# lz4/lz4-java

Measured on NVIDIA H100. Metric: lz4_fast_compress_plus_decompress_64KiB_blocks, higher is better.
Workload: dtype u8

## Files before the change

lz4-java_b200/csrc/lz4_decompress.cu:

```cuda
#include "common.cuh"
#include "kernels.h"

namespace b200 {

#ifndef B200_DEC_MINB_BATCH
#define B200_DEC_MINB_BATCH 8
#endif
#ifndef B200_DEC_WIN
#define B200_DEC_WIN 512
#endif
static constexpr int DEC_WIN = B200_DEC_WIN;

struct VarLen { uint32_t len; int ip; bool err; };

__device__ __forceinline__ VarLen read_varlen(const uint8_t* __restrict__ src, int ip, int ilimit, bool initial_check)
{
    VarLen r; r.len = 0; r.ip = ip; r.err = false;
    if (initial_check && ip >= ilimit) { r.err = true; return r; }
    uint32_t s;
    do {
        s = src[r.ip]; r.ip++;
        r.len = min(r.len + s, 0x40000000u);
        if (r.ip > ilimit) { r.err = true; return r; }
    } while (s == 255);
    return r;
}

__device__ __forceinline__ void lane_copy16(uint8_t* d, const uint8_t* s, int n)
{
    const uintptr_t sa = reinterpret_cast<uintptr_t>(s);
    const uint32_t* w = reinterpret_cast<const uint32_t*>(sa & ~uintptr_t(3));
    const uint32_t sh = (uint32_t(sa) & 3u) * 8u;
    uint32_t x[5];
    #pragma unroll
    for (int t = 0; t < 5; t++) x[t] = (4 * t < n + 3) ? w[t] : 0u;
    #pragma unroll
    for (int t = 0; t < 4; t++) {
        const uint32_t v = __funnelshift_r(x[t], x[t + 1], sh);
        if (4 * t     < n) d[4 * t]     = uint8_t(v);
        if (4 * t + 1 < n) d[4 * t + 1] = uint8_t(v >> 8);
        if (4 * t + 2 < n) d[4 * t + 2] = uint8_t(v >> 16);
        if (4 * t + 3 < n) d[4 * t + 3] = uint8_t(v >> 24);
    }
}

__device__ __forceinline__ int decode_batch(const uint8_t* __restrict__ src, uint8_t* dst, int& ip, int& op,
                                            const int iend, const int oend, const int lane, uint8_t* win)
{
    const uint8_t* __restrict__ in = src + ip;
    uint8_t* cls = win + DEC_WIN;
    {
        const uintptr_t base = reinterpret_cast<uintptr_t>(in);
        const uint32_t* __restrict__ W = reinterpret_cast<const uint32_t*>(base & ~uintptr_t(3)) + 4 * lane;
        const uint32_t a8 = (uint32_t(base) & 3u) * 8u;
        const uint32_t w0 = W[0], w1 = W[1], w2 = W[2], w3 = W[3], w4 = W[4];
        uint32_t f[4];
        f[0] = __funnelshift_r(w0, w1, a8); f[1] = __funnelshift_r(w1, w2, a8); f[2] = __funnelshift_r(w2, w3, a8); f[3] = __funnelshift_r(w3, w4, a8);
        uint32_t c[4];
        #pragma unroll
        for (int k = 0; k < 4; k++) {
            const uint32_t t = f[k];
            const uint32_t lit = (t >> 4) & 0x0F0F0F0Fu, ml = t & 0x0F0F0F0Fu;
            const uint32_t m15 = ((ml + 0x01010101u) >> 4) & 0x01010101u;
            c[k] = (lit + 0x03030303u) | (m15 << 5);
        }
        __syncwarp();
        reinterpret_cast<uint4*>(win)[lane] = make_uint4(f[0], f[1], f[2], f[3]);
        reinterpret_cast<uint4*>(cls)[lane] = make_uint4(c[0], c[1], c[2], c[3]);
        __syncwarp();
    }
    auto wbyte = [&](int p) -> uint32_t { return p < DEC_WIN ? win[p] : in[p]; };
    const int ilim = iend - ip - 64;
    const int olim = oend - op - 128;

    int k = 0, q = 0;
    int m_tok = 0;
    while (k < 32 && q < DEC_WIN - 8) {
        const int c = cls[q];
        int s = c & 31;
        if (c > 17) {
            bool ok = true;
            if (s == 18) {
                int p = q + 1, lit = 15; uint32_t e;
                do { if (p >= ilim) { ok = false; break; } e = wbyte(p++); lit += int(e); } while (e == 255u && lit < (1 << 24));
                s = (p - q) + lit + 2;
                ok = ok && lit < (1 << 24);
            }
            if (ok && (c & 32)) {
                uint32_t e; int cnt = 0;
                do { if (q + s >= ilim) { ok = false; break; } e = wbyte(q + s); s++; } while (e == 255u && ++cnt < (1 << 16));
                ok = ok && cnt < (1 << 16);
            }
            if (!ok || q + s > ilim) break;
        }
        if (lane == k) m_tok = q;
        q += s; k++;
    }
    if (k == 0) return 0;
    int m_lit = 0, m_ml = 0, m_lsrc = 0;
    if (lane < k) {
        const uint32_t tok = win[m_tok];
        m_lit = int(tok >> 4); m_ml = int(tok & 15u) + 4; m_lsrc = m_tok + 1;
        if (m_lit == 15) { uint32_t e; do { e = wbyte(m_lsrc++); m_lit += int(e); } while (e == 255u); }
        if (m_ml == 19) { int p = m_lsrc + m_lit + 2; uint32_t e; do { e = wbyte(p++); m_ml += int(e); } while (e == 255u); }
    }
    int m_out = m_lit + m_ml;
    #pragma unroll
    for (int d = 1; d < 32; d <<= 1) { const int y = __shfl_up_sync(B200_FULL, m_out, d); if (lane >= d) m_out += y; }
    {
        const unsigned over = __ballot_sync(B200_FULL, lane < k && m_out > olim);
        if (over) {
            k = __ffs(over) - 1;
            if (k == 0) return 0;
            q = __shfl_sync(B200_FULL, m_tok, k);
        }
    }
    int acc = __shfl_sync(B200_FULL, m_out, k - 1);
    m_out -= m_lit + m_ml;
    if (lane >= k) { m_lit = 0; m_ml = 0; }

    int off = 1;
    if (lane < k) off = int(in[m_lsrc + m_lit]) | (int(in[m_lsrc + m_lit + 1]) << 8);
    const int mstart = op + m_out + m_lit;
    const unsigned bad = __ballot_sync(B200_FULL, lane < k && (off == 0 || off > mstart));
    if (bad) {
        k = __ffs(bad) - 1;
        if (k == 0) return 0;
        acc = __shfl_sync(B200_FULL, m_out, k);
        q = __shfl_sync(B200_FULL, m_tok, k);
    }
    const bool mine = lane < k;

    if (mine) lane_copy16(dst + op + m_out, in + m_lsrc, min(m_lit, 16));
    if (__any_sync(B200_FULL, mine && m_lit > 16)) {
        if (mine && m_lit > 16) lane_copy16(dst + op + m_out + 16, in + m_lsrc + 16, min(m_lit - 16, 16));
        for (unsigned lm = __ballot_sync(B200_FULL, mine && m_lit > 32); lm; lm &= lm - 1) {
            const int j = __ffs(lm) - 1;
            const int jo = __shfl_sync(B200_FULL, m_out, j), js = __shfl_sync(B200_FULL, m_lsrc, j), jl = __shfl_sync(B200_FULL, m_lit, j);
            warp_copy(dst + op + jo + 32, in + js + 32, jl - 32, lane);
        }
    }
    __syncwarp();

    const bool ovl = off < m_ml;
    const int mend = mstart - off + m_ml;
    unsigned pend = k == 32 ? B200_FULL : (1u << k) - 1u;
    while (pend) {
        const int fp = __ffs(pend) - 1;
        const int fpm = __shfl_sync(B200_FULL, mstart, fp);
        if (__shfl_sync(B200_FULL, int(ovl), fp)) {
            warp_match_copy(dst + fpm, __shfl_sync(B200_FULL, off, fp), __shfl_sync(B200_FULL, m_ml, fp), lane);
            pend &= pend - 1;
            __syncwarp();
            continue;
        }
        const bool ready = ((pend >> lane) & 1u) && !ovl && (lane == fp || mend <= fpm);
        const unsigned rm = __ballot_sync(B200_FULL, ready);
        if (ready) lane_copy16(dst + mstart, dst + mstart - off, min(m_ml, 16));
        if (__any_sync(B200_FULL, ready && m_ml > 16)) {
            if (ready && m_ml > 16) lane_copy16(dst + mstart + 16, dst + mstart - off + 16, min(m_ml - 16, 16));
            for (unsigned lm = __ballot_sync(B200_FULL, ready && m_ml > 32); lm; lm &= lm - 1) {
                const int j = __ffs(lm) - 1;
                const int jm = __shfl_sync(B200_FULL, mstart, j), jo = __shfl_sync(B200_FULL, off, j), jl = __shfl_sync(B200_FULL, m_ml, j);
                warp_copy(dst + jm + 32, dst + jm - jo + 32, jl - 32, lane);
            }
        }
        pend &= ~rm;
        __syncwarp();
    }
    ip += q; op += acc;
    return k;
}

template <int WARPS, bool BATCH>
__global__ void __launch_bounds__(WARPS * 32, BATCH ? B200_DEC_MINB_BATCH : 2048 / (WARPS * 32))
lz4_decompress_safe_kernel(const uint8_t* __restrict__ src_base, const uint64_t* __restrict__ src_off,
                           const int32_t* __restrict__ src_len,
                           uint8_t* dst_base, const uint64_t* __restrict__ dst_off,
                           const int32_t* __restrict__ dst_cap, int32_t* __restrict__ result, uint32_t n)
{
    __shared__ __align__(16) uint8_t s_win[BATCH ? WARPS : 1][2 * DEC_WIN];
    uint8_t* win = s_win[BATCH ? (threadIdx.x >> 5) : 0];
    const uint32_t b = blockIdx.x * WARPS + (threadIdx.x >> 5);
    if (b >= n) return;
    const int lane = lane_id();
    const uint8_t* __restrict__ src = src_base + src_off[b];
    uint8_t* dst = dst_base + dst_off[b];
    const int iend = src_len[b];
    const int oend = dst_cap[b];
    int ip = 0, op = 0;
    int ret;

    if (oend < 0) { ret = -1; goto done; }
    if (oend == 0) { ret = (iend == 1 && src[0] == 0) ? 0 : -1; goto done; }
    if (iend <= 0) { ret = -1; goto done; }
    {
        bool fastloop = oend >= 64;
        const uint8_t* __restrict__ sl = src + lane;
        uint8_t* dl = dst + lane;
        for (;;) {
            while (BATCH && fastloop && ip + DEC_WIN + 128 <= iend && op + 256 <= oend) { if (decode_batch(src, dst, ip, op, iend, oend, lane, win) == 0) break; }
            while (fastloop && ip + 18 <= iend) {
                const uint32_t token = src[ip];
                const uint32_t lit = token >> 4, mlc = token & 15;
                if (lit == 15 || mlc == 15) break;
                if (lane < lit) dl[op] = sl[ip + 1];
                const int ipo = ip + 1 + (int)lit;
                const uint32_t off = (uint32_t)src[ipo] | ((uint32_t)src[ipo + 1] << 8);
                const int op2 = op + (int)lit, ml = (int)mlc + 4;
                if (op2 + ml >= oend - 64 || off > (uint32_t)op2 || off == 0) break;
                __syncwarp();
                if (off >= (uint32_t)ml) { if (lane < ml) dl[op2] = dl[op2 - (int)off]; }
                else warp_match_copy(dst + op2, (int)off, ml, lane);
                ip = ipo + 2; op = op2 + ml;
            }
            const uint32_t token = src[ip++];
            uint32_t len = token >> 4;
            bool apply_end_rule, shortcut = false;
            if (fastloop) {
                bool leave;
                if (len == 15) {
                    VarLen v = read_varlen(src, ip, iend - 15, true);
                    ip = v.ip; if (v.err) goto error;
                    len += v.len;
                    leave = ((long long)op + len > oend - 32) || ((long long)ip + len > iend - 32);
                } else leave = ip > iend - 17;
                if (leave) fastloop = false;
                apply_end_rule = leave;
            } else {
                shortcut = (len != 15) && (ip < iend - 16) && (op <= oend - 32);
                if (!shortcut && len == 15) {
                    VarLen v = read_varlen(src, ip, iend - 15, true);
                    ip = v.ip; if (v.err) goto error;
                    len += v.len;
                }
                apply_end_rule = !shortcut;
            }
            const long long lcpy = (long long)op + len;
            if (apply_end_rule && (lcpy > oend - 12 || (long long)ip + len > iend - 8)) {
                if ((long long)ip + len != iend || lcpy > oend) goto error;
                warp_copy(dst + op, src + ip, (int)len, lane);
                op += (int)len;
                break;
            }
            warp_copy(dst + op, src + ip, (int)len, lane);
            ip += (int)len; op += (int)len;

            const int off = src[ip] | (src[ip + 1] << 8);
            ip += 2;
            uint32_t ml = token & 15;
            const bool direct = shortcut && ml != 15 && off >= 8 && off <= op;
            if (ml == 15) {
                VarLen v = read_varlen(src, ip, iend - 4, false);
                ip = v.ip; if (v.err) goto error;
                ml += v.len;
            }
            ml += 4;
            if (!direct) {
                if (off > op) goto error;
                const long long mcpy = (long long)op + ml;
                if (fastloop && mcpy >= oend - 64) fastloop = false;
                if (mcpy > oend - 5) goto error;
            }
            __syncwarp();
            if (off == 0) {
                for (int i = lane; i < (int)ml; i += 32) dst[op + i] = 0;
            } else {
                warp_match_copy(dst + op, off, (int)ml, lane);
            }
            op += (int)ml;
        }
        ret = op;
        goto done;
    }
error:
    ret = -ip - 1;
done:
    __syncwarp();
    if (lane == 0) { __threadfence(); result[b] = ret; }
}

template <int WARPS, bool BATCH>
__global__ void __launch_bounds__(WARPS * 32, BATCH ? B200_DEC_MINB_BATCH : 2048 / (WARPS * 32))
lz4_decompress_fast_kernel(const uint8_t* __restrict__ src_base, const uint64_t* __restrict__ src_off,
                           const int32_t* __restrict__ src_avail,
                           uint8_t* dst_base, const uint64_t* __restrict__ dst_off,
                           const int32_t* __restrict__ dst_len, int32_t* __restrict__ result, uint32_t n)
{
    __shared__ __align__(16) uint8_t s_win[BATCH ? WARPS : 1][2 * DEC_WIN];
    uint8_t* win = s_win[BATCH ? (threadIdx.x >> 5) : 0];
    const uint32_t b = blockIdx.x * WARPS + (threadIdx.x >> 5);
    if (b >= n) return;
    const int lane = lane_id();
    const uint8_t* __restrict__ src = src_base + src_off[b];
    uint8_t* dst = dst_base + dst_off[b];
    const int avail = src_avail[b];
    const int oend = dst_len[b];
    int ip = 0, op = 0, ret = -1;

    if (oend < 0) goto done;
    for (;;) {
        while (BATCH && ip + DEC_WIN + 128 <= avail && op + 256 <= oend) { if (decode_batch(src, dst, ip, op, avail, oend, lane, win) == 0) break; }
        {
            const uint8_t* __restrict__ sl = src + lane;
            uint8_t* dl = dst + lane;
            while (ip + 17 <= avail) {
                const uint32_t token = src[ip];
                const uint32_t lit = token >> 4, mlc = token & 15;
                if (lit == 15 || mlc == 15) break;
                const int op2 = op + (int)lit, ml = (int)mlc + 4;
                if (op2 + 23 > oend) break;
                if (lane < lit) dl[op] = sl[ip + 1];
                const int ipo = ip + 1 + (int)lit;
                const uint32_t off = (uint32_t)src[ipo] | ((uint32_t)src[ipo + 1] << 8);
                if (off > (uint32_t)op2 || off == 0) break;
                __syncwarp();
                if (off >= (uint32_t)ml) { if (lane < ml) dl[op2] = dl[op2 - (int)off]; }
                else warp_match_copy(dst + op2, (int)off, ml, lane);
                ip = ipo + 2; op = op2 + ml;
            }
        }
        if (ip >= avail) goto done;
        const uint32_t token = src[ip++];
        uint32_t ll = token >> 4;
        if (ll == 15) {
            uint32_t s;
            do { if (ip >= avail) goto done; s = src[ip++]; ll = min(ll + s, 0x40000000u); } while (s == 255);
        }
        if ((uint32_t)(oend - op) < ll) goto done;
        if ((long long)ip + ll > avail) goto done;
        warp_copy(dst + op, src + ip, (int)ll, lane);
        op += (int)ll; ip += (int)ll;
        if (oend - op < 12) {
            if (op == oend) { ret = ip; }
            goto done;
        }
        if (ip + 2 > avail) goto done;
        const int off = src[ip] | (src[ip + 1] << 8);
        ip += 2;
        uint32_t ml = token & 15;
        if (ml == 15) {
            uint32_t s;
            do { if (ip >= avail) goto done; s = src[ip++]; ml = min(ml + s, 0x40000000u); } while (s == 255);
        }
        ml += 4;
        if ((uint32_t)(oend - op) < ml) goto done;
        if (off > op) goto done;
        __syncwarp();
        if (off != 0) warp_match_copy(dst + op, off, (int)ml, lane);
        else for (int i = lane; i < (int)ml; i += 32) dst[op + i] = 0;
        op += (int)ml;
        if (oend - op < 5) goto done;
    }
done:
    if (lane == 0) result[b] = ret;
}

#ifndef B200_HOST_SIM
static constexpr int DEC_WARPS = 4;

cudaError_t launch_decompress_safe(const BatchArgs& a, cudaStream_t st)
{
    if (a.n == 0) return cudaSuccess;
    const unsigned grid = (unsigned)((a.n + DEC_WARPS - 1) / DEC_WARPS);
    lz4_decompress_safe_kernel<DEC_WARPS, true><<<grid, DEC_WARPS * 32, 0, st>>>(
        a.src_base, a.src_off, a.src_len, a.dst_base, a.dst_off, a.dst_cap, a.result, (uint32_t)a.n);
    return cudaGetLastError();
}

cudaError_t launch_decompress_fast(const BatchArgs& a, cudaStream_t st)
{
    if (a.n == 0) return cudaSuccess;
    const unsigned grid = (unsigned)((a.n + DEC_WARPS - 1) / DEC_WARPS);
    lz4_decompress_fast_kernel<DEC_WARPS, true><<<grid, DEC_WARPS * 32, 0, st>>>(
        a.src_base, a.src_off, a.src_len, a.dst_base, a.dst_off, a.dst_cap, a.result, (uint32_t)a.n);
    return cudaGetLastError();
}

#endif

}
```

lz4-java_b200/csrc/xxhash.cu:

```cuda
#include "common.cuh"
#include "kernels.h"

namespace b200 {

static constexpr uint32_t P32_1 = 2654435761u, P32_2 = 2246822519u, P32_3 = 3266489917u,
                          P32_4 = 668265263u, P32_5 = 374761393u;
static constexpr uint64_t P64_1 = 11400714785074694791ull, P64_2 = 14029467366897019727ull,
                          P64_3 = 1609587929392839161ull, P64_4 = 9650029242287828579ull,
                          P64_5 = 2870177450012600261ull;

__device__ __forceinline__ uint32_t rotl32(uint32_t x, int r) { return __funnelshift_l(x, x, r); }
__device__ __forceinline__ uint64_t rotl64(uint64_t x, int r) { return (x << r) | (x >> (64 - r)); }
__device__ __forceinline__ uint32_t round32(uint32_t acc, uint32_t w) { return rotl32(acc + w * P32_2, 13) * P32_1; }
__device__ __forceinline__ uint64_t round64(uint64_t acc, uint64_t w) { return rotl64(acc + w * P64_2, 31) * P64_1; }
__device__ __forceinline__ uint64_t merge64(uint64_t h, uint64_t v) { return (h ^ round64(0, v)) * P64_1 + P64_4; }

__device__ __forceinline__ uint64_t load_u64_unaligned(const uint8_t* p)
{
    return uint64_t(load_u32_unaligned(p)) | (uint64_t(load_u32_unaligned(p + 4)) << 32);
}

__device__ __forceinline__ uint32_t finish32(uint32_t h, const uint8_t* p, uint32_t rem)
{
    while (rem >= 4) { h = rotl32(h + load_u32_unaligned(p) * P32_3, 17) * P32_4; p += 4; rem -= 4; }
    while (rem)      { h = rotl32(h + uint32_t(*p++) * P32_5, 11) * P32_1; rem--; }
    h ^= h >> 15; h *= P32_2; h ^= h >> 13; h *= P32_3; h ^= h >> 16;
    return h;
}
__device__ __forceinline__ uint64_t finish64(uint64_t h, const uint8_t* p, uint32_t rem)
{
    while (rem >= 8) { h = rotl64(h ^ round64(0, load_u64_unaligned(p)), 27) * P64_1 + P64_4; p += 8; rem -= 8; }
    if (rem >= 4)    { h = rotl64(h ^ (uint64_t(load_u32_unaligned(p)) * P64_1), 23) * P64_2 + P64_3; p += 4; rem -= 4; }
    while (rem)      { h = rotl64(h ^ (uint64_t(*p++) * P64_5), 11) * P64_1; rem--; }
    h ^= h >> 33; h *= P64_2; h ^= h >> 29; h *= P64_3; h ^= h >> 32;
    return h;
}

#ifndef B200_HOST_SIM
__device__ __forceinline__ uint32_t smem_u32(const void* p) { return (uint32_t)__cvta_generic_to_shared(p); }
__device__ __forceinline__ void mbar_init(uint32_t bar, uint32_t count)
{ asm volatile("mbarrier.init.shared::cta.b64 [%0], %1;" :: "r"(bar), "r"(count) : "memory"); }
__device__ __forceinline__ void mbar_arrive_expect_tx(uint32_t bar, uint32_t bytes)
{ asm volatile("mbarrier.arrive.expect_tx.shared::cta.b64 _, [%0], %1;" :: "r"(bar), "r"(bytes) : "memory"); }
__device__ __forceinline__ void mbar_wait(uint32_t bar, uint32_t parity)
{
    uint32_t ok;
    do {
        asm volatile("{\n\t.reg .pred p;\n\tmbarrier.try_wait.parity.shared::cta.b64 p, [%1], %2;\n\tselp.u32 %0, 1, 0, p;\n\t}"
                     : "=r"(ok) : "r"(bar), "r"(parity) : "memory");
    } while (!ok);
}
__device__ __forceinline__ void tma_bulk_g2s(uint32_t dst_smem, const void* src_gmem, uint32_t bytes, uint32_t bar)
{
    asm volatile("cp.async.bulk.shared::cluster.global.mbarrier::complete_tx::bytes [%0], [%1], %2, [%3];"
                 :: "r"(dst_smem), "l"(src_gmem), "r"(bytes), "r"(bar) : "memory");
}

#endif

template <int BITS> struct XxhTraits;
template <> struct XxhTraits<32> { using word = uint32_t; static constexpr int STRIPE = 16; };
template <> struct XxhTraits<64> { using word = uint64_t; static constexpr int STRIPE = 32; };

template <int BITS> struct Acc;
template <> struct Acc<32> {
    uint32_t v1, v2, v3, v4;
    __device__ __forceinline__ void init(uint32_t seed) { v1 = seed + P32_1 + P32_2; v2 = seed + P32_2; v3 = seed; v4 = seed - P32_1; }
    __device__ __forceinline__ void stripe(uint4 q) { v1 = round32(v1, q.x); v2 = round32(v2, q.y); v3 = round32(v3, q.z); v4 = round32(v4, q.w); }
    __device__ __forceinline__ void stripe_g(const uint8_t* p) {
        stripe(make_uint4(load_u32_unaligned(p), load_u32_unaligned(p + 4), load_u32_unaligned(p + 8), load_u32_unaligned(p + 12)));
    }
    __device__ __forceinline__ uint32_t merge() const { return rotl32(v1, 1) + rotl32(v2, 7) + rotl32(v3, 12) + rotl32(v4, 18); }
};
template <> struct Acc<64> {
    uint64_t v1, v2, v3, v4;
    __device__ __forceinline__ void init(uint64_t seed) { v1 = seed + P64_1 + P64_2; v2 = seed + P64_2; v3 = seed; v4 = seed - P64_1; }
    __device__ __forceinline__ void stripe(uint4 a, uint4 b) {
        v1 = round64(v1, uint64_t(a.x) | (uint64_t(a.y) << 32)); v2 = round64(v2, uint64_t(a.z) | (uint64_t(a.w) << 32));
        v3 = round64(v3, uint64_t(b.x) | (uint64_t(b.y) << 32)); v4 = round64(v4, uint64_t(b.z) | (uint64_t(b.w) << 32));
    }
    __device__ __forceinline__ void stripe_g(const uint8_t* p) {
        v1 = round64(v1, load_u64_unaligned(p)); v2 = round64(v2, load_u64_unaligned(p + 8));
        v3 = round64(v3, load_u64_unaligned(p + 16)); v4 = round64(v4, load_u64_unaligned(p + 24));
    }
    __device__ __forceinline__ uint64_t merge() const {
        uint64_t h = rotl64(v1, 1) + rotl64(v2, 7) + rotl64(v3, 12) + rotl64(v4, 18);
        h = merge64(h, v1); h = merge64(h, v2); h = merge64(h, v3); h = merge64(h, v4);
        return h;
    }
};

#ifndef B200_HOST_SIM
static constexpr int XXH_WARPS = 4;
static constexpr int XXH_CHUNK = 256;
static constexpr int XXH_SLOT  = XXH_CHUNK + 16;
static constexpr int XXH_STAGES = 2;
static constexpr size_t XXH_SMEM = size_t(XXH_WARPS) * XXH_STAGES * 32 * XXH_SLOT + 64;

template <int BITS>
__global__ void __launch_bounds__(XXH_WARPS * 32)
xxh_batch_kernel(const uint8_t* __restrict__ base, const uint64_t* __restrict__ off, const int32_t* __restrict__ len,
                 typename XxhTraits<BITS>::word seed, typename XxhTraits<BITS>::word* __restrict__ out, uint32_t n)
{
    using word = typename XxhTraits<BITS>::word;
    constexpr int STRIPE = XxhTraits<BITS>::STRIPE;
    extern __shared__ __align__(128) uint8_t smem[];
    const int warp = threadIdx.x >> 5, lane = lane_id();
    const uint32_t first = (blockIdx.x * XXH_WARPS + warp) * 32;
    if (first >= n) return;
    const uint32_t i = first + lane;
    const bool live = i < n;

    const uint8_t* p = live ? base + off[i] : base;
    const uint32_t L = live ? (uint32_t)max(len[i], 0) : 0u;
    const uint32_t bulk = L & ~uint32_t(STRIPE - 1);
    Acc<BITS> acc; acc.init(seed);

    uint64_t* bars = reinterpret_cast<uint64_t*>(smem);
    uint8_t* slots = smem + 64 + size_t(warp) * XXH_STAGES * 32 * XXH_SLOT;
    const bool aligned = (reinterpret_cast<uintptr_t>(p) & 15) == 0 || bulk == 0;

    if (__all_sync(B200_FULL, aligned)) {
        const uint32_t bar0 = smem_u32(&bars[warp * XXH_STAGES]);
        if (lane == 0) {
            for (int s = 0; s < XXH_STAGES; s++) mbar_init(bar0 + 8 * s, 1);
            asm volatile("fence.mbarrier_init.release.cluster;" ::: "memory");
        }
        __syncwarp();
        const uint32_t nchunks = (bulk + XXH_CHUNK - 1) / XXH_CHUNK;
        const uint32_t maxchunks = __reduce_max_sync(B200_FULL, nchunks);

        auto issue = [&](uint32_t k) {
            const uint32_t s = k % XXH_STAGES;
            const uint32_t bytes = k < nchunks ? min(uint32_t(XXH_CHUNK), bulk - k * XXH_CHUNK) : 0u;
            const uint32_t total = __reduce_add_sync(B200_FULL, bytes);
            if (lane == 0) mbar_arrive_expect_tx(bar0 + 8 * s, total);
            if (bytes) tma_bulk_g2s(smem_u32(slots + (size_t(s) * 32 + lane) * XXH_SLOT), p + size_t(k) * XXH_CHUNK, bytes, bar0 + 8 * s);
        };
        for (uint32_t k = 0; k < XXH_STAGES && k < maxchunks; k++) issue(k);
        for (uint32_t k = 0; k < maxchunks; k++) {
            const uint32_t s = k % XXH_STAGES;
            mbar_wait(bar0 + 8 * s, (k / XXH_STAGES) & 1);
            if (k < nchunks) {
                const uint32_t bytes = min(uint32_t(XXH_CHUNK), bulk - k * XXH_CHUNK);
                const uint4* q = reinterpret_cast<const uint4*>(slots + (size_t(s) * 32 + lane) * XXH_SLOT);
                if constexpr (BITS == 32) {
                    #pragma unroll 4
                    for (uint32_t j = 0; j < bytes / 16; j++) acc.stripe(q[j]);
                } else {
                    #pragma unroll 4
                    for (uint32_t j = 0; j < bytes / 32; j++) acc.stripe(q[2 * j], q[2 * j + 1]);
                }
            }
            __syncwarp();
            if (k + XXH_STAGES < maxchunks) issue(k + XXH_STAGES);
        }
    } else {
        for (uint32_t o = 0; o < bulk; o += STRIPE) acc.stripe_g(p + o);
    }

    if (live) {
        if constexpr (BITS == 32) {
            uint32_t h = (L >= 16u) ? acc.merge() : seed + P32_5;
            out[i] = finish32(h + L, p + bulk, L - bulk);
        } else {
            uint64_t h = (L >= 32u) ? acc.merge() : seed + P64_5;
            out[i] = finish64(h + uint64_t(L), p + bulk, L - bulk);
        }
    }
}

cudaError_t launch_xxh32(const uint8_t* base, const uint64_t* off, const int32_t* len, uint32_t seed,
                         uint32_t* out, size_t n, cudaStream_t st)
{
    if (n == 0) return cudaSuccess;
    auto k = xxh_batch_kernel<32>;
    cudaError_t e = cudaFuncSetAttribute(k, cudaFuncAttributeMaxDynamicSharedMemorySize, (int)XXH_SMEM);
    if (e != cudaSuccess) return e;
    const unsigned grid = (unsigned)((n + XXH_WARPS * 32 - 1) / (XXH_WARPS * 32));
    k<<<grid, XXH_WARPS * 32, XXH_SMEM, st>>>(base, off, len, seed, out, (uint32_t)n);
    return cudaGetLastError();
}

cudaError_t launch_xxh64(const uint8_t* base, const uint64_t* off, const int32_t* len, uint64_t seed,
                         uint64_t* out, size_t n, cudaStream_t st)
{
    if (n == 0) return cudaSuccess;
    auto k = xxh_batch_kernel<64>;
    cudaError_t e = cudaFuncSetAttribute(k, cudaFuncAttributeMaxDynamicSharedMemorySize, (int)XXH_SMEM);
    if (e != cudaSuccess) return e;
    const unsigned grid = (unsigned)((n + XXH_WARPS * 32 - 1) / (XXH_WARPS * 32));
    k<<<grid, XXH_WARPS * 32, XXH_SMEM, st>>>(base, off, len, seed, out, (uint32_t)n);
    return cudaGetLastError();
}

#endif

__device__ __forceinline__ uint32_t xxh32_chain_init(uint32_t seed, int lane)
{
    const int c = lane & 3;
    return c == 0 ? seed + P32_1 + P32_2 : c == 1 ? seed + P32_2 : c == 2 ? seed : seed - P32_1;
}

template <bool CG>
__device__ __forceinline__ uint32_t xxh_ldw(const uint32_t* p)
{
#ifndef B200_HOST_SIM
    if constexpr (CG) return __ldcg(p);
#endif
    return *p;
}

template <bool CG = false>
__device__ __forceinline__ uint32_t xxh32_warp_rows(uint32_t v, const uint8_t* __restrict__ p, size_t rows, int lane)
{
    constexpr int R = 8;
    const uintptr_t sa = reinterpret_cast<uintptr_t>(p);
    const uint32_t* __restrict__ W = reinterpret_cast<const uint32_t*>(sa & ~uintptr_t(3));
    const uint32_t sh = (uint32_t(sa) & 3u) * 8u;
    const int c = lane & 3;
    auto ldrow = [&](size_t r) -> uint32_t {
        const size_t i = r * 32 + lane;
        const uint32_t a = xxh_ldw<CG>(W + i);
        return sh ? __funnelshift_r(a, xxh_ldw<CG>(W + i + 1), sh) : a;
    };
    uint32_t cur[R], nxt[R];
    const size_t groups = rows / R;
    if (groups) {
        #pragma unroll
        for (int r = 0; r < R; r++) cur[r] = ldrow(r);
    }
    for (size_t g = 0; g < groups; g++) {
        if (g + 1 < groups) {
            #pragma unroll
            for (int r = 0; r < R; r++) nxt[r] = ldrow((g + 1) * R + r);
        }
        #pragma unroll
        for (int r = 0; r < R; r++) {
            #pragma unroll
            for (int st = 0; st < 8; st++) v = round32(v, __shfl_sync(B200_FULL, cur[r], 4 * st + c));
        }
        #pragma unroll
        for (int r = 0; r < R; r++) cur[r] = nxt[r];
    }
    for (size_t r = groups * R; r < rows; r++) {
        const uint32_t x = ldrow(r);
        #pragma unroll
        for (int st = 0; st < 8; st++) v = round32(v, __shfl_sync(B200_FULL, x, 4 * st + c));
    }
    return v;
}

template <bool CG = false>
__device__ __forceinline__ uint32_t xxh32_warp_stripes(uint32_t v, const uint8_t* __restrict__ p, size_t stripes, int lane)
{
    const size_t rows = stripes >> 3;
    v = xxh32_warp_rows<CG>(v, p, rows, lane);
    for (size_t t = rows << 3; t < stripes; t++) {
        const uint8_t* q = p + 16 * t + 4 * (lane & 3);
        if constexpr (CG) {
            const uintptr_t a = reinterpret_cast<uintptr_t>(q);
            const uint32_t* w = reinterpret_cast<const uint32_t*>(a & ~uintptr_t(3));
            const uint32_t sh = (uint32_t(a) & 3u) * 8u;
            const uint32_t lo = xxh_ldw<true>(w);
            v = round32(v, sh ? __funnelshift_r(lo, xxh_ldw<true>(w + 1), sh) : lo);
        } else {
            v = round32(v, load_u32_unaligned(q));
        }
    }
    return v;
}

__device__ __forceinline__ uint32_t xxh32_chain_merge(uint32_t v)
{
    return rotl32(__shfl_sync(B200_FULL, v, 0), 1) + rotl32(__shfl_sync(B200_FULL, v, 1), 7) +
           rotl32(__shfl_sync(B200_FULL, v, 2), 12) + rotl32(__shfl_sync(B200_FULL, v, 3), 18);
}

__global__ void __launch_bounds__(32)
xxh32_long_kernel(const uint8_t* __restrict__ base, const uint64_t* __restrict__ off, const int32_t* __restrict__ len,
                  uint32_t seed, uint32_t* __restrict__ out, uint32_t n)
{
    const uint32_t i = blockIdx.x;
    if (i >= n) return;
    const int lane = lane_id();
    const uint8_t* __restrict__ p = base + off[i];
    const uint32_t L = (uint32_t)max(len[i], 0);
    const size_t stripes = L >> 4;
    uint32_t h;
    if (L >= 16u) h = xxh32_chain_merge(xxh32_warp_stripes(xxh32_chain_init(seed, lane), p, stripes, lane));
    else h = seed + P32_5;
    if (lane == 0) out[i] = finish32(h + L, p + 16 * stripes, L & 15u);
}

#ifndef B200_HOST_SIM
cudaError_t launch_xxh32_long(const uint8_t* base, const uint64_t* off, const int32_t* len, uint32_t seed,
                              uint32_t* out, size_t n, cudaStream_t st)
{
    if (n == 0) return cudaSuccess;
    xxh32_long_kernel<<<(unsigned)n, 32, 0, st>>>(base, off, len, seed, out, (uint32_t)n);
    return cudaGetLastError();
}
#endif

__global__ void __launch_bounds__(32)
xxh32_long_carry_kernel(const uint8_t* __restrict__ base, const uint64_t* __restrict__ off, const uint64_t* __restrict__ len,
                        uint32_t* __restrict__ out, Xxh32Carry* __restrict__ c_state, const uint8_t* __restrict__ c_mode, uint32_t n)
{
    __shared__ __align__(16) uint8_t s_mem[16];
    const uint32_t r = blockIdx.x;
    if (r >= n) return;
    const int lane = lane_id();
    const uint32_t mode = c_mode[r];
    const uint8_t* __restrict__ p = base + off[r];
    uint64_t L = len[r];
    uint32_t v = xxh32_chain_init(0u, lane), mem = 0;
    uint64_t total = 0;
    if (mode & XXH_CARRY_IN) {
        const Xxh32Carry& c = c_state[r];
        v = c.v[lane & 3]; total = c.total; mem = c.memsize;
        if (uint32_t(lane) < mem) s_mem[lane] = c.mem[lane];
    }
    __syncwarp();
    total += L;
    if (mem + L < 16u) {
        if (uint32_t(lane) < L) s_mem[mem + lane] = p[lane];
        mem += (uint32_t)L; L = 0;
    } else {
        if (mem) {
            const uint32_t t = 16u - mem;
            if (uint32_t(lane) < t) s_mem[mem + lane] = p[lane];
            __syncwarp();
            v = round32(v, reinterpret_cast<const uint32_t*>(s_mem)[lane & 3]);
            p += t; L -= t; mem = 0;
            __syncwarp();
        }
        const size_t stripes = size_t(L >> 4);
        v = xxh32_warp_stripes(v, p, stripes, lane);
        mem = uint32_t(L & 15u);
        if (uint32_t(lane) < mem) s_mem[lane] = p[16 * stripes + lane];
    }
    __syncwarp();
    if (mode & XXH_CARRY_OUT) {
        Xxh32Carry& c = c_state[r];
        if (lane < 4) c.v[lane] = v;
        if (uint32_t(lane) < mem) c.mem[lane] = s_mem[lane];
        if (lane == 0) { c.total = total; c.memsize = mem; }
        return;
    }
    const uint32_t h = total >= 16 ? xxh32_chain_merge(v) : 0u + P32_5;
    if (lane == 0) out[r] = finish32(h + uint32_t(total), s_mem, mem);
}

cudaError_t launch_xxh32_long_carry(const uint8_t* base, const uint64_t* off, const uint64_t* len, uint32_t* out, Xxh32Carry* carry,
                                    const uint8_t* mode, size_t n, cudaStream_t st)
{
    if (n == 0) return cudaSuccess;
    B200_LAUNCH(xxh32_long_carry_kernel, (unsigned)n, 32, st, base, off, len, out, carry, mode, (uint32_t)n);
    return cudaGetLastError();
}

__device__ __forceinline__ uint8_t ld_byte_l2(const uint8_t* p)
{
#ifndef B200_HOST_SIM
    return __ldcg(p);
#else
    return *p;
#endif
}

__global__ void __launch_bounds__(32)
xxh32_frames_chained_kernel(const uint8_t* __restrict__ slots, const uint64_t* __restrict__ blk_off, const uint32_t* __restrict__ f_first,
                            const uint32_t* __restrict__ f_nblk, const int32_t* __restrict__ blk_comp, const int32_t* __restrict__ blk_rawlen,
                            const int32_t* c_res, uint32_t* __restrict__ out, uint32_t n, Xxh32Carry* c_state = nullptr,
                            const uint8_t* c_mode = nullptr)
{
    __shared__ __align__(16) uint8_t s_carry[16];
    const uint32_t f = blockIdx.x;
    if (f >= n) return;
    const int lane = lane_id();
    const uint32_t first = f_first[f], nblk = f_nblk[f];
    const uint32_t mode = c_mode ? c_mode[f] : 0u;
    uint32_t v = xxh32_chain_init(0u, lane);
    uint64_t total = 0; uint32_t carry = 0;
    bool big = false;
    if (mode & XXH_CARRY_IN) {
        const Xxh32Carry& c = c_state[f];
        v = c.v[lane & 3]; total = c.total; carry = c.memsize; big = total >= 16;
        if (uint32_t(lane) < carry) s_carry[lane] = c.mem[lane];
        __syncwarp();
    }
    for (uint32_t k = 0; k < nblk; k++) {
        const int32_t ci = blk_comp[first + k];
        int32_t r;
        if (ci < 0) r = blk_rawlen[first + k];
        else {
            const volatile int32_t* w = c_res + ci;
            r = 0;
            if (lane == 0) { while ((r = *w) == FRAME_RES_PENDING) { B200_NANOSLEEP(256); } }
            r = __shfl_sync(B200_FULL, r, 0);
            __threadfence();
            if (r < 0) break;
        }
        const uint8_t* p = slots + blk_off[first + k];
        uint32_t len = uint32_t(r);
        total += len;
        if (carry) {
            const uint32_t t = min(16u - carry, len);
            if (uint32_t(lane) < t) s_carry[carry + lane] = ld_byte_l2(p + lane);
            __syncwarp();
            carry += t; p += t; len -= t;
            if (carry < 16u) continue;
            v = round32(v, reinterpret_cast<const uint32_t*>(s_carry)[lane & 3]); big = true; carry = 0;
            __syncwarp();
        }
        const size_t stripes = size_t(len) >> 4;
        if (stripes) { v = xxh32_warp_stripes<true>(v, p, stripes, lane); big = true; }
        carry = len & 15u;
        if (uint32_t(lane) < carry) s_carry[lane] = ld_byte_l2(p + 16 * stripes + lane);
        __syncwarp();
    }
    if (mode & XXH_CARRY_OUT) {
        Xxh32Carry& c = c_state[f];
        if (lane < 4) c.v[lane] = v;
        if (uint32_t(lane) < carry) c.mem[lane] = s_carry[lane];
        if (lane == 0) { c.total = total; c.memsize = carry; }
        return;
    }
    const uint32_t h = big ? xxh32_chain_merge(v) : 0u + P32_5;
    if (lane == 0) out[f] = finish32(h + uint32_t(total), s_carry, carry);
}

#ifndef B200_HOST_SIM
cudaError_t launch_xxh32_frames_chained(const uint8_t* slots, const uint64_t* blk_off, const uint32_t* f_first, const uint32_t* f_nblk,
                                        const int32_t* blk_comp, const int32_t* blk_rawlen, const int32_t* c_res,
                                        uint32_t* out, size_t n, cudaStream_t st)
{
    if (n == 0) return cudaSuccess;
    xxh32_frames_chained_kernel<<<(unsigned)n, 32, 0, st>>>(slots, blk_off, f_first, f_nblk, blk_comp, blk_rawlen, c_res, out, (uint32_t)n);
    return cudaGetLastError();
}
#endif
cudaError_t launch_xxh32_frames_chained_carry(const uint8_t* slots, const uint64_t* blk_off, const uint32_t* f_first,
                                              const uint32_t* f_nblk, const int32_t* blk_comp, const int32_t* blk_rawlen,
                                              const int32_t* c_res, uint32_t* out, size_t n, Xxh32Carry* carry,
                                              const uint8_t* mode, cudaStream_t st)
{
    if (n == 0) return cudaSuccess;
    B200_LAUNCH(xxh32_frames_chained_kernel, (unsigned)n, 32, st, slots, blk_off, f_first, f_nblk, blk_comp, blk_rawlen, c_res, out,
                (uint32_t)n, carry, mode);
    return cudaGetLastError();
}

__device__ __forceinline__ uint64_t xxh64_chain_init(uint64_t seed, int lane)
{
    const int c = lane & 3;
    return c == 0 ? seed + P64_1 + P64_2 : c == 1 ? seed + P64_2 : c == 2 ? seed : seed - P64_1;
}

__device__ __forceinline__ uint64_t xxh64_warp_rows(uint64_t v, const uint8_t* __restrict__ p, size_t rows, int lane)
{
    constexpr int R = 4;
    const uintptr_t sa = reinterpret_cast<uintptr_t>(p);
    const uint32_t* __restrict__ W = reinterpret_cast<const uint32_t*>(sa & ~uintptr_t(3));
    const uint32_t sh = (uint32_t(sa) & 3u) * 8u;
    const int c = lane & 3;
    auto ldrow = [&](size_t r) -> uint2 {
        const size_t i = (r * 32 + lane) * 2;
        const uint32_t a = W[i], b = W[i + 1];
        if (!sh) return make_uint2(a, b);
        return make_uint2(__funnelshift_r(a, b, sh), __funnelshift_r(b, W[i + 2], sh));
    };
    auto feed = [&](uint2 x) {
        #pragma unroll
        for (int st = 0; st < 8; st++) {
            const uint32_t lo = __shfl_sync(B200_FULL, x.x, 4 * st + c), hi = __shfl_sync(B200_FULL, x.y, 4 * st + c);
            v = round64(v, uint64_t(lo) | (uint64_t(hi) << 32));
        }
    };
    uint2 cur[R], nxt[R];
    const size_t groups = rows / R;
    if (groups) {
        #pragma unroll
        for (int r = 0; r < R; r++) cur[r] = ldrow(r);
    }
    for (size_t g = 0; g < groups; g++) {
        if (g + 1 < groups) {
            #pragma unroll
            for (int r = 0; r < R; r++) nxt[r] = ldrow((g + 1) * R + r);
        }
        #pragma unroll
        for (int r = 0; r < R; r++) feed(cur[r]);
        #pragma unroll
        for (int r = 0; r < R; r++) cur[r] = nxt[r];
    }
    for (size_t r = groups * R; r < rows; r++) feed(ldrow(r));
    return v;
}

__device__ __forceinline__ uint64_t xxh64_warp_stripes(uint64_t v, const uint8_t* __restrict__ p, size_t stripes, int lane)
{
    const size_t rows = stripes >> 3;
    v = xxh64_warp_rows(v, p, rows, lane);
    for (size_t t = rows << 3; t < stripes; t++) v = round64(v, load_u64_unaligned(p + 32 * t + 8 * (lane & 3)));
    return v;
}

__device__ __forceinline__ uint64_t shfl_u64(uint64_t x, int src)
{
    return uint64_t(__shfl_sync(B200_FULL, uint32_t(x), src)) | (uint64_t(__shfl_sync(B200_FULL, uint32_t(x >> 32), src)) << 32);
}

__device__ __forceinline__ uint64_t xxh64_chain_merge(uint64_t v)
{
    const uint64_t v1 = shfl_u64(v, 0), v2 = shfl_u64(v, 1), v3 = shfl_u64(v, 2), v4 = shfl_u64(v, 3);
    uint64_t h = rotl64(v1, 1) + rotl64(v2, 7) + rotl64(v3, 12) + rotl64(v4, 18);
    h = merge64(h, v1); h = merge64(h, v2); h = merge64(h, v3); h = merge64(h, v4);
    return h;
}

__global__ void __launch_bounds__(32)
xxh64_long_kernel(const uint8_t* __restrict__ base, const uint64_t* __restrict__ off, const int32_t* __restrict__ len,
                  uint64_t seed, uint64_t* __restrict__ out, uint32_t n)
{
    const uint32_t i = blockIdx.x;
    if (i >= n) return;
    const int lane = lane_id();
    const uint8_t* __restrict__ p = base + off[i];
    const uint32_t L = (uint32_t)max(len[i], 0);
    const size_t stripes = L >> 5;
    uint64_t h;
    if (L >= 32u) h = xxh64_chain_merge(xxh64_warp_stripes(xxh64_chain_init(seed, lane), p, stripes, lane));
    else h = seed + P64_5;
    if (lane == 0) out[i] = finish64(h + uint64_t(L), p + 32 * stripes, L & 31u);
}

#ifndef B200_HOST_SIM
cudaError_t launch_xxh64_long(const uint8_t* base, const uint64_t* off, const int32_t* len, uint64_t seed,
                              uint64_t* out, size_t n, cudaStream_t st)
{
    if (n == 0) return cudaSuccess;
    xxh64_long_kernel<<<(unsigned)n, 32, 0, st>>>(base, off, len, seed, out, (uint32_t)n);
    return cudaGetLastError();
}
#endif

__global__ void xxh32_stream_kernel(Xxh32State* s, int op, uint32_t seed, const uint8_t* __restrict__ p, size_t len)
{
    const int lane = lane_id();
    if (op == XXH_OP_RESET) {
        if (lane) return;
        s->total = 0; s->memsize = 0; s->seed = seed;
        s->v[0] = seed + P32_1 + P32_2; s->v[1] = seed + P32_2; s->v[2] = seed; s->v[3] = seed - P32_1;
        return;
    }
    if (op == XXH_OP_UPDATE) {
        const uint32_t memsize = s->memsize;
        const uint64_t total = s->total;
        uint32_t v = s->v[lane & 3];
        __syncwarp();
        if (memsize + len < 16) {
            if (lane == 0) { for (size_t i = 0; i < len; i++) s->mem[memsize + i] = p[i]; s->memsize = memsize + (uint32_t)len; s->total = total + len; }
            return;
        }
        if (memsize) {
            const uint32_t fill = 16 - memsize;
            if (lane == 0) for (uint32_t i = 0; i < fill; i++) s->mem[memsize + i] = p[i];
            __syncwarp();
            v = round32(v, load_u32_unaligned(s->mem + 4 * (lane & 3)));
            p += fill; len -= fill;
            __syncwarp();
        }
        const size_t stripes = len >> 4;
        v = xxh32_warp_stripes(v, p, stripes, lane);
        if (lane < 4) s->v[lane] = v;
        if (lane == 0) {
            const uint32_t r = (uint32_t)(len & 15);
            for (uint32_t i = 0; i < r; i++) s->mem[i] = p[16 * stripes + i];
            s->memsize = r; s->total = total + (memsize ? 16 - memsize : 0) + len;
        }
        return;
    }
    if (lane) return;
    {
        uint32_t h;
        if (s->total >= 16) h = rotl32(s->v[0], 1) + rotl32(s->v[1], 7) + rotl32(s->v[2], 12) + rotl32(s->v[3], 18);
        else h = s->seed + P32_5;
        h += (uint32_t)s->total;
        s->digest = finish32(h, s->mem, s->memsize);
    }
}

__global__ void xxh64_stream_kernel(Xxh64State* s, int op, uint64_t seed, const uint8_t* __restrict__ p, size_t len)
{
    const int lane = lane_id();
    if (op == XXH_OP_RESET) {
        if (lane) return;
        s->total = 0; s->memsize = 0; s->seed = seed;
        s->v[0] = seed + P64_1 + P64_2; s->v[1] = seed + P64_2; s->v[2] = seed; s->v[3] = seed - P64_1;
        return;
    }
    if (op == XXH_OP_UPDATE) {
        const uint32_t memsize = s->memsize;
        const uint64_t total = s->total;
        uint64_t v = s->v[lane & 3];
        __syncwarp();
        if (memsize + len < 32) {
            if (lane == 0) { for (size_t i = 0; i < len; i++) s->mem[memsize + i] = p[i]; s->memsize = memsize + (uint32_t)len; s->total = total + len; }
            return;
        }
        if (memsize) {
            const uint32_t fill = 32 - memsize;
            if (lane == 0) for (uint32_t i = 0; i < fill; i++) s->mem[memsize + i] = p[i];
            __syncwarp();
            v = round64(v, load_u64_unaligned(s->mem + 8 * (lane & 3)));
            p += fill; len -= fill;
            __syncwarp();
        }
        const size_t stripes = len >> 5;
        v = xxh64_warp_stripes(v, p, stripes, lane);
        if (lane < 4) s->v[lane] = v;
        if (lane == 0) {
            const uint32_t r = (uint32_t)(len & 31);
            for (uint32_t i = 0; i < r; i++) s->mem[i] = p[32 * stripes + i];
            s->memsize = r; s->total = total + (memsize ? 32 - memsize : 0) + len;
        }
        return;
    }
    if (lane) return;
    {
        uint64_t h;
        if (s->total >= 32) {
            h = rotl64(s->v[0], 1) + rotl64(s->v[1], 7) + rotl64(s->v[2], 12) + rotl64(s->v[3], 18);
            for (int k = 0; k < 4; k++) h = merge64(h, s->v[k]);
        } else h = s->seed + P64_5;
        h += s->total;
        s->digest = finish64(h, s->mem, s->memsize);
    }
}

#ifndef B200_HOST_SIM
cudaError_t launch_xxh32_stream(Xxh32State* st, int op, uint32_t seed, const uint8_t* data, size_t len, cudaStream_t s)
{
    xxh32_stream_kernel<<<1, 32, 0, s>>>(st, op, seed, data, len);
    return cudaGetLastError();
}
cudaError_t launch_xxh64_stream(Xxh64State* st, int op, uint64_t seed, const uint8_t* data, size_t len, cudaStream_t s)
{
    xxh64_stream_kernel<<<1, 32, 0, s>>>(st, op, seed, data, len);
    return cudaGetLastError();
}
#endif

}
```

Baseline: 76.55.

## Add decompress trace probes and grid-stride the chained xxh32 frame kernel

Adds compile-time-gated clock64 tracing to the batch decoder that records per-phase cycle counts, which is off by default. Separately, the chained xxh32 frame kernel now uses a grid-stride loop with a grid capped at four blocks per SM instead of one block per frame. This bounds the number of spin-waiting blocks that poll for compression results and cuts launch size. The risk is less parallelism when there are many frames, and extra host calls to query the SM count on every launch.

```diff
diff --git a/lz4-java_b200/csrc/lz4_decompress.cu b/lz4-java_b200/csrc/lz4_decompress.cu
--- a/lz4-java_b200/csrc/lz4_decompress.cu
+++ b/lz4-java_b200/csrc/lz4_decompress.cu
@@ -12,6 +12,32 @@
 static constexpr int DEC_WIN = B200_DEC_WIN;
 
 struct VarLen { uint32_t len; int ip; bool err; };
+
+#ifdef B200_DEC_TRACE
+enum { DT_TOTAL, DT_WINDOW, DT_WALK, DT_LIT, DT_MATCH, DT_BATCHES, DT_SEQUENCES, DT_ROUNDS, DT_OVERLAPPING,
+       DT_SEQUENTIAL, DT_N, DT_LAST = DT_N };
+constexpr int DEC_TRACE_EVERY = 64, DEC_TRACE_ROWS = 16384;
+__device__ unsigned long long g_dec_trace[DEC_TRACE_ROWS][DT_N];
+#define DT_PARAM , unsigned long long* dt
+#define DT_ARG , dt
+#define DT_BEGIN unsigned long long dt[DT_N + 1] = {}; const long long dt_start = clock64()
+#define DT_START (dt[DT_LAST] = clock64())
+#define DT_MARK(slot) do { const unsigned long long t_ = clock64(); dt[slot] += t_ - dt[DT_LAST]; dt[DT_LAST] = t_; } while (0)
+#define DT_ADD(slot, v) (dt[slot] += (v))
+#define DT_END do {                                                                                                  \
+        if (lane == 0 && b % DEC_TRACE_EVERY == 0 && b / DEC_TRACE_EVERY < DEC_TRACE_ROWS) {                         \
+            dt[DT_TOTAL] = clock64() - dt_start;                                                                     \
+            for (int i_ = 0; i_ < DT_N; i_++) g_dec_trace[b / DEC_TRACE_EVERY][i_] = dt[i_];                         \
+        } } while (0)
+#else
+#define DT_PARAM
+#define DT_ARG
+#define DT_BEGIN
+#define DT_START
+#define DT_MARK(slot)
+#define DT_ADD(slot, v)
+#define DT_END
+#endif
 
 __device__ __forceinline__ VarLen read_varlen(const uint8_t* __restrict__ src, int ip, int ilimit, bool initial_check)
 {
@@ -45,8 +71,9 @@
 }
 
 __device__ __forceinline__ int decode_batch(const uint8_t* __restrict__ src, uint8_t* dst, int& ip, int& op,
-                                            const int iend, const int oend, const int lane, uint8_t* win)
-{
+                                            const int iend, const int oend, const int lane, uint8_t* win DT_PARAM)
+{
+    DT_START;
     const uint8_t* __restrict__ in = src + ip;
     uint8_t* cls = win + DEC_WIN;
     {
@@ -69,6 +96,7 @@
         reinterpret_cast<uint4*>(cls)[lane] = make_uint4(c[0], c[1], c[2], c[3]);
         __syncwarp();
     }
+    DT_MARK(DT_WINDOW);
     auto wbyte = [&](int p) -> uint32_t { return p < DEC_WIN ? win[p] : in[p]; };
     const int ilim = iend - ip - 64;
     const int olim = oend - op - 128;
@@ -96,7 +124,7 @@
         if (lane == k) m_tok = q;
         q += s; k++;
     }
-    if (k == 0) return 0;
+    if (k == 0) { DT_MARK(DT_WALK); return 0; }
     int m_lit = 0, m_ml = 0, m_lsrc = 0;
     if (lane < k) {
         const uint32_t tok = win[m_tok];
@@ -111,7 +139,7 @@
         const unsigned over = __ballot_sync(B200_FULL, lane < k && m_out > olim);
         if (over) {
             k = __ffs(over) - 1;
-            if (k == 0) return 0;
+            if (k == 0) { DT_MARK(DT_WALK); return 0; }
             q = __shfl_sync(B200_FULL, m_tok, k);
         }
     }
@@ -125,11 +153,12 @@
     const unsigned bad = __ballot_sync(B200_FULL, lane < k && (off == 0 || off > mstart));
     if (bad) {
         k = __ffs(bad) - 1;
-        if (k == 0) return 0;
+        if (k == 0) { DT_MARK(DT_WALK); return 0; }
         acc = __shfl_sync(B200_FULL, m_out, k);
         q = __shfl_sync(B200_FULL, m_tok, k);
     }
     const bool mine = lane < k;
+    DT_MARK(DT_WALK);
 
     if (mine) lane_copy16(dst + op + m_out, in + m_lsrc, min(m_lit, 16));
     if (__any_sync(B200_FULL, mine && m_lit > 16)) {
@@ -141,11 +170,14 @@
         }
     }
     __syncwarp();
+    DT_MARK(DT_LIT);
 
     const bool ovl = off < m_ml;
     const int mend = mstart - off + m_ml;
     unsigned pend = k == 32 ? B200_FULL : (1u << k) - 1u;
+    DT_ADD(DT_OVERLAPPING, __popc(__ballot_sync(B200_FULL, mine && off < m_ml)));
     while (pend) {
+        DT_ADD(DT_ROUNDS, 1);
         const int fp = __ffs(pend) - 1;
         const int fpm = __shfl_sync(B200_FULL, mstart, fp);
         if (__shfl_sync(B200_FULL, int(ovl), fp)) {
@@ -169,6 +201,8 @@
         __syncwarp();
     }
     ip += q; op += acc;
+    DT_MARK(DT_MATCH);
+    DT_ADD(DT_BATCHES, 1); DT_ADD(DT_SEQUENCES, k);
     return k;
 }
 
@@ -184,6 +218,7 @@
     const uint32_t b = blockIdx.x * WARPS + (threadIdx.x >> 5);
     if (b >= n) return;
     const int lane = lane_id();
+    DT_BEGIN;
     const uint8_t* __restrict__ src = src_base + src_off[b];
     uint8_t* dst = dst_base + dst_off[b];
     const int iend = src_len[b];
@@ -199,7 +234,7 @@
         const uint8_t* __restrict__ sl = src + lane;
         uint8_t* dl = dst + lane;
         for (;;) {
-            while (BATCH && fastloop && ip + DEC_WIN + 128 <= iend && op + 256 <= oend) { if (decode_batch(src, dst, ip, op, iend, oend, lane, win) == 0) break; }
+            while (BATCH && fastloop && ip + DEC_WIN + 128 <= iend && op + 256 <= oend) { if (decode_batch(src, dst, ip, op, iend, oend, lane, win DT_ARG) == 0) break; }
             while (fastloop && ip + 18 <= iend) {
                 const uint32_t token = src[ip];
                 const uint32_t lit = token >> 4, mlc = token & 15;
@@ -209,12 +244,14 @@
                 const uint32_t off = (uint32_t)src[ipo] | ((uint32_t)src[ipo + 1] << 8);
                 const int op2 = op + (int)lit, ml = (int)mlc + 4;
                 if (op2 + ml >= oend - 64 || off > (uint32_t)op2 || off == 0) break;
+                DT_ADD(DT_SEQUENTIAL, 1);
                 __syncwarp();
                 if (off >= (uint32_t)ml) { if (lane < ml) dl[op2] = dl[op2 - (int)off]; }
                 else warp_match_copy(dst + op2, (int)off, ml, lane);
                 ip = ipo + 2; op = op2 + ml;
             }
             const uint32_t token = src[ip++];
+            DT_ADD(DT_SEQUENTIAL, 1);
             uint32_t len = token >> 4;
             bool apply_end_rule, shortcut = false;
             if (fastloop) {
@@ -277,6 +314,7 @@
     ret = -ip - 1;
 done:
     __syncwarp();
+    DT_END;
     if (lane == 0) { __threadfence(); result[b] = ret; }
 }
 
@@ -292,6 +330,7 @@
     const uint32_t b = blockIdx.x * WARPS + (threadIdx.x >> 5);
     if (b >= n) return;
     const int lane = lane_id();
+    DT_BEGIN;
     const uint8_t* __restrict__ src = src_base + src_off[b];
     uint8_t* dst = dst_base + dst_off[b];
     const int avail = src_avail[b];
@@ -300,7 +339,7 @@
 
     if (oend < 0) goto done;
     for (;;) {
-        while (BATCH && ip + DEC_WIN + 128 <= avail && op + 256 <= oend) { if (decode_batch(src, dst, ip, op, avail, oend, lane, win) == 0) break; }
+        while (BATCH && ip + DEC_WIN + 128 <= avail && op + 256 <= oend) { if (decode_batch(src, dst, ip, op, avail, oend, lane, win DT_ARG) == 0) break; }
         {
             const uint8_t* __restrict__ sl = src + lane;
             uint8_t* dl = dst + lane;
@@ -314,6 +353,7 @@
                 const int ipo = ip + 1 + (int)lit;
                 const uint32_t off = (uint32_t)src[ipo] | ((uint32_t)src[ipo + 1] << 8);
                 if (off > (uint32_t)op2 || off == 0) break;
+                DT_ADD(DT_SEQUENTIAL, 1);
                 __syncwarp();
                 if (off >= (uint32_t)ml) { if (lane < ml) dl[op2] = dl[op2 - (int)off]; }
                 else warp_match_copy(dst + op2, (int)off, ml, lane);
@@ -322,6 +362,7 @@
         }
         if (ip >= avail) goto done;
         const uint32_t token = src[ip++];
+        DT_ADD(DT_SEQUENTIAL, 1);
         uint32_t ll = token >> 4;
         if (ll == 15) {
             uint32_t s;
@@ -353,11 +394,20 @@
         if (oend - op < 5) goto done;
     }
 done:
+    DT_END;
     if (lane == 0) result[b] = ret;
 }
 
 #ifndef B200_HOST_SIM
 static constexpr int DEC_WARPS = 4;
+
+#ifdef B200_DEC_TRACE
+extern "C" int b200lz4_dec_trace_read(unsigned long long* host, int rows)
+{
+    if (rows < 0 || rows > DEC_TRACE_ROWS) return -1;
+    return cudaMemcpyFromSymbol(host, g_dec_trace, size_t(rows) * DT_N * sizeof(unsigned long long)) == cudaSuccess ? DT_N : -1;
+}
+#endif
 
 cudaError_t launch_decompress_safe(const BatchArgs& a, cudaStream_t st)
 {
diff --git a/lz4-java_b200/csrc/xxhash.cu b/lz4-java_b200/csrc/xxhash.cu
--- a/lz4-java_b200/csrc/xxhash.cu
+++ b/lz4-java_b200/csrc/xxhash.cu
@@ -376,59 +376,76 @@
                             const uint8_t* c_mode = nullptr)
 {
     __shared__ __align__(16) uint8_t s_carry[16];
-    const uint32_t f = blockIdx.x;
-    if (f >= n) return;
     const int lane = lane_id();
-    const uint32_t first = f_first[f], nblk = f_nblk[f];
-    const uint32_t mode = c_mode ? c_mode[f] : 0u;
-    uint32_t v = xxh32_chain_init(0u, lane);
-    uint64_t total = 0; uint32_t carry = 0;
-    bool big = false;
-    if (mode & XXH_CARRY_IN) {
-        const Xxh32Carry& c = c_state[f];
-        v = c.v[lane & 3]; total = c.total; carry = c.memsize; big = total >= 16;
-        if (uint32_t(lane) < carry) s_carry[lane] = c.mem[lane];
+    for (uint32_t f = blockIdx.x; f < n; f += gridDim.x) {
+        const uint32_t first = f_first[f], nblk = f_nblk[f];
+        const uint32_t mode = c_mode ? c_mode[f] : 0u;
+        uint32_t v = xxh32_chain_init(0u, lane);
+        uint64_t total = 0; uint32_t carry = 0;
+        bool big = false;
+        if (mode & XXH_CARRY_IN) {
+            const Xxh32Carry& c = c_state[f];
+            v = c.v[lane & 3]; total = c.total; carry = c.memsize; big = total >= 16;
+            if (uint32_t(lane) < carry) s_carry[lane] = c.mem[lane];
+            __syncwarp();
+        }
+        for (uint32_t k = 0; k < nblk; k++) {
+            const int32_t ci = blk_comp[first + k];
+            int32_t r;
+            if (ci < 0) r = blk_rawlen[first + k];
+            else {
+                const volatile int32_t* w = c_res + ci;
+                r = 0;
+                if (lane == 0) { while ((r = *w) == FRAME_RES_PENDING) { B200_NANOSLEEP(256); } }
+                r = __shfl_sync(B200_FULL, r, 0);
+                __threadfence();
+                if (r < 0) break;
+            }
+            const uint8_t* p = slots + blk_off[first + k];
+            uint32_t len = uint32_t(r);
+            total += len;
+            if (carry) {
+                const uint32_t t = min(16u - carry, len);
+                if (uint32_t(lane) < t) s_carry[carry + lane] = ld_byte_l2(p + lane);
+                __syncwarp();
+                carry += t; p += t; len -= t;
+                if (carry < 16u) continue;
+                v = round32(v, reinterpret_cast<const uint32_t*>(s_carry)[lane & 3]); big = true; carry = 0;
+                __syncwarp();
+            }
+            const size_t stripes = size_t(len) >> 4;
+            if (stripes) { v = xxh32_warp_stripes<true>(v, p, stripes, lane); big = true; }
+            carry = len & 15u;
+            if (uint32_t(lane) < carry) s_carry[lane] = ld_byte_l2(p + 16 * stripes + lane);
+            __syncwarp();
+        }
+        if (mode & XXH_CARRY_OUT) {
+            Xxh32Carry& c = c_state[f];
+            if (lane < 4) c.v[lane] = v;
+            if (uint32_t(lane) < carry) c.mem[lane] = s_carry[lane];
+            if (lane == 0) { c.total = total; c.memsize = carry; }
+        } else {
+            const uint32_t h = big ? xxh32_chain_merge(v) : 0u + P32_5;
+            if (lane == 0) out[f] = finish32(h + uint32_t(total), s_carry, carry);
+        }
         __syncwarp();
     }
-    for (uint32_t k = 0; k < nblk; k++) {
-        const int32_t ci = blk_comp[first + k];
-        int32_t r;
-        if (ci < 0) r = blk_rawlen[first + k];
-        else {
-            const volatile int32_t* w = c_res + ci;
-            r = 0;
-            if (lane == 0) { while ((r = *w) == FRAME_RES_PENDING) { B200_NANOSLEEP(256); } }
-            r = __shfl_sync(B200_FULL, r, 0);
-            __threadfence();
-            if (r < 0) break;
-        }
-        const uint8_t* p = slots + blk_off[first + k];
-        uint32_t len = uint32_t(r);
-        total += len;
-        if (carry) {
-            const uint32_t t = min(16u - carry, len);
-            if (uint32_t(lane) < t) s_carry[carry + lane] = ld_byte_l2(p + lane);
-            __syncwarp();
-            carry += t; p += t; len -= t;
-            if (carry < 16u) continue;
-            v = round32(v, reinterpret_cast<const uint32_t*>(s_carry)[lane & 3]); big = true; carry = 0;
-            __syncwarp();
-        }
-        const size_t stripes = size_t(len) >> 4;
-        if (stripes) { v = xxh32_warp_stripes<true>(v, p, stripes, lane); big = true; }
-        carry = len & 15u;
-        if (uint32_t(lane) < carry) s_carry[lane] = ld_byte_l2(p + 16 * stripes + lane);
-        __syncwarp();
-    }
-    if (mode & XXH_CARRY_OUT) {
-        Xxh32Carry& c = c_state[f];
-        if (lane < 4) c.v[lane] = v;
-        if (uint32_t(lane) < carry) c.mem[lane] = s_carry[lane];
-        if (lane == 0) { c.total = total; c.memsize = carry; }
-        return;
-    }
-    const uint32_t h = big ? xxh32_chain_merge(v) : 0u + P32_5;
-    if (lane == 0) out[f] = finish32(h + uint32_t(total), s_carry, carry);
+}
+
+static constexpr int XXH_CHAINED_PER_SM = 4;
+
+static cudaError_t chained_grid(size_t n, unsigned& grid)
+{
+#ifdef B200_HOST_SIM
+    grid = (unsigned)min(n, size_t(XXH_CHAINED_PER_SM));
+    return cudaSuccess;
+#else
+    int dev = 0, sms = 0;
+    cudaError_t e = cudaGetDevice(&dev);
+    if (e == cudaSuccess) e = cudaDeviceGetAttribute(&sms, cudaDevAttrMultiProcessorCount, dev);
+    grid = (unsigned)min(n, size_t(sms > 0 ? sms : 1) * XXH_CHAINED_PER_SM);
+    return e;
+#endif
 }
 
 #ifndef B200_HOST_SIM
@@ -437,7 +454,9 @@
                                         uint32_t* out, size_t n, cudaStream_t st)
 {
     if (n == 0) return cudaSuccess;
-    xxh32_frames_chained_kernel<<<(unsigned)n, 32, 0, st>>>(slots, blk_off, f_first, f_nblk, blk_comp, blk_rawlen, c_res, out, (uint32_t)n);
+    unsigned grid;
+    if (cudaError_t e = chained_grid(n, grid)) return e;
+    xxh32_frames_chained_kernel<<<grid, 32, 0, st>>>(slots, blk_off, f_first, f_nblk, blk_comp, blk_rawlen, c_res, out, (uint32_t)n);
     return cudaGetLastError();
 }
 #endif
@@ -447,7 +466,9 @@
                                               const uint8_t* mode, cudaStream_t st)
 {
     if (n == 0) return cudaSuccess;
-    B200_LAUNCH(xxh32_frames_chained_kernel, (unsigned)n, 32, st, slots, blk_off, f_first, f_nblk, blk_comp, blk_rawlen, c_res, out,
+    unsigned grid;
+    if (cudaError_t e = chained_grid(n, grid)) return e;
+    B200_LAUNCH(xxh32_frames_chained_kernel, grid, 32, st, slots, blk_off, f_first, f_nblk, blk_comp, blk_rawlen, c_res, out,
                 (uint32_t)n, carry, mode);
     return cudaGetLastError();
 }
```

Measured after the change: 76.78, median of 6. Within noise of the previous version (+0.3%).
